# EdwardjkFeng/gradslam

Hardware: AMD Instinct MI355X
Metric: RGB-D frames/sec (640x480, 10 ICP iters) (higher is better)
Workload: dtype f32; 1 GPU; c2: ICP odometry localisation step, 640x480 TUM-shape synthetic RGB-D, batch 1 per GPU, dsratio 4 (~19k x ~19k points), 10 LM iterations, map 288269 points; parallelism=one sequence per GPU, final RCCL all_gather of poses, timing=one timed region of 1356 steps

## Files before the change

gradslam_amd/csrc/gs_icp_assoc.hpp:

```cpp
#pragma once

#include <type_traits>

#include "gs_common.hpp"

namespace gs {

constexpr int KNN_T = 256;
constexpr int KNN_NW = 16;
constexpr int KNN_BT = KNN_NW * 64;
constexpr int KNN_COARSE = 512;
constexpr int CHUNK = 16;
constexpr int WROWS = 3;
constexpr int WBANDS = WROWS + 1;
constexpr int SUPER = 64;
constexpr int KNN_LIST = 4096;
constexpr int NACC = 29;
constexpr int LIN_T = 256;
constexpr int LIN_MAXB = 1024;
constexpr unsigned long long KEY_NONE = ~0ull;

__device__ __forceinline__ unsigned long long pack_key(float d, int j) {
    return ((unsigned long long)fbits(d) << 32) | (unsigned int)j;
}
__device__ __forceinline__ float dist2(f3 s, float tx, float ty, float tz) {
    const float dx = s.x - tx, dy = s.y - ty, dz = s.z - tz;
    return (dx * dx + dy * dy) + dz * dz;
}

struct Row {
    float a[6], b;
    bool valid;
};

__device__ __forceinline__ Row make_row(const float *__restrict__ src, const float *__restrict__ tgt,
                                        const float *__restrict__ nrm, const unsigned long long *__restrict__ best,
                                        int i, int ns, float thresh) {
    Row r;
    r.valid = false;
    if (i >= ns) return r;
    const unsigned long long key = best[i];
    if (key == KEY_NONE) return r;
    const uint32_t j = (uint32_t)(key & 0xffffffffu);
    const float d2 = bitsf((uint32_t)(key >> 32));
    if (thresh >= 0.0f && !(d2 < thresh)) return r;
    const f3 s = ld3(src, i), d = ld3(tgt, j), n = ld3(nrm, j);
    r.a[0] = n.x; r.a[1] = n.y; r.a[2] = n.z;
    r.a[3] = n.z * s.y - n.y * s.z;
    r.a[4] = n.x * s.z - n.z * s.x;
    r.a[5] = n.y * s.x - n.x * s.y;
    r.b = (n.x * (d.x - s.x) + n.y * (d.y - s.y)) + n.z * (d.z - s.z);
    r.valid = true;
    return r;
}

__device__ __forceinline__ void accumulate_row(const Row &r, float *acc) {
    int q = 0;
#pragma unroll
    for (int u = 0; u < 6; ++u)
#pragma unroll
        for (int v = u; v < 6; ++v) { acc[q] = __fmaf_rn(r.a[u], r.a[v], acc[q]); ++q; }
#pragma unroll
    for (int u = 0; u < 6; ++u) acc[21 + u] = __fmaf_rn(r.a[u], r.b, acc[21 + u]);
    acc[27] = __fmaf_rn(r.b, r.b, acc[27]);
    acc[28] += 1.0f;
}

__device__ __forceinline__ Row make_row_from(const f3 s, const bool ok, const unsigned long long key,
                                             const float *__restrict__ tgt, const float *__restrict__ nrm, float thresh) {
    Row r;
    r.valid = false;
    if (!ok || key == KEY_NONE) return r;
    const uint32_t j = (uint32_t)(key & 0xffffffffu);
    const float d2 = bitsf((uint32_t)(key >> 32));
    if (thresh >= 0.0f && !(d2 < thresh)) return r;
    const f3 d = ld3(tgt, j), n = ld3(nrm, j);
    r.a[0] = n.x; r.a[1] = n.y; r.a[2] = n.z;
    r.a[3] = n.z * s.y - n.y * s.z;
    r.a[4] = n.x * s.z - n.z * s.x;
    r.a[5] = n.y * s.x - n.x * s.y;
    r.b = (n.x * (d.x - s.x) + n.y * (d.y - s.y)) + n.z * (d.z - s.z);
    r.valid = true;
    return r;
}

constexpr int POOL = 4096;

struct CamK {
    float R[9], T[3], fx, fy, cx, cy;
    int ds, Wd, Hd;
};
struct KnnShared {
    unsigned long long key[64];
    int cnt;
    float tbox[6];
    int win[WROWS][64];
    int wflag[64];
    int centre[64];
    CamK cam;
    int band[2 * WBANDS + 1];
    int plan[2 * WBANDS];
    unsigned int plan_ready;
    float seed[2][64][4];
    union alignas(16) {
        struct {
            int list[KNN_LIST];
            float rows[NACC][65];
            float part[NACC][16];
        } a;
        float stage[POOL * 4];
    } u;
};

__device__ unsigned int g_loop_counts[4];

#ifdef GS_DIAG_STAMPS
__device__ unsigned long long *g_diag = nullptr;
#define GS_STAMP(slot)                                                                                   \
    do {                                                                                                 \
        if (g_diag && (threadIdx.x & 63) == 0)                                                           \
            g_diag[((size_t)blockIdx.x * KNN_NW + (threadIdx.x >> 6)) * 16 + (slot)] = wall_clock64();   \
    } while (0)
#define GS_COUNT(slot, v)                                                                                \
    do {                                                                                                 \
        if (g_diag && (threadIdx.x & 63) == 0)                                                           \
            g_diag[((size_t)blockIdx.x * KNN_NW + (threadIdx.x >> 6)) * 16 + (slot)] = (v);             \
    } while (0)
#define GS_TICK(var) const unsigned int var = (unsigned int)wall_clock64()
#define GS_ACCUM(acc, t0) acc += (unsigned int)wall_clock64() - (t0)
#else
#define GS_STAMP(slot)
#define GS_COUNT(slot, v)
#define GS_TICK(var)
#define GS_ACCUM(acc, t0)
#endif

__device__ __forceinline__ float rlane(float v, int l) {
    return __int_as_float(__builtin_amdgcn_readlane(__float_as_int(v), l));
}
template <int CTRL>
__device__ __forceinline__ int dpp_i(int v) {
    return __builtin_amdgcn_update_dpp(v, v, CTRL, 0xf, 0xf, false);
}
template <class Op>
__device__ __forceinline__ int wave_reduce_i(int v, Op op) {
    v = op(v, dpp_i<0xB1>(v));
    v = op(v, dpp_i<0x4E>(v));
    v = op(v, dpp_i<0x141>(v));
    v = op(v, dpp_i<0x140>(v));
    return op(op(__builtin_amdgcn_readlane(v, 0), __builtin_amdgcn_readlane(v, 16)),
              op(__builtin_amdgcn_readlane(v, 32), __builtin_amdgcn_readlane(v, 48)));
}
template <class Op>
__device__ __forceinline__ float wave_reduce_f(float v, Op op) {
    auto d = [](float x, auto tag) { return __int_as_float(dpp_i<decltype(tag)::value>(__float_as_int(x))); };
    v = op(v, d(v, std::integral_constant<int, 0xB1>{}));
    v = op(v, d(v, std::integral_constant<int, 0x4E>{}));
    v = op(v, d(v, std::integral_constant<int, 0x141>{}));
    v = op(v, d(v, std::integral_constant<int, 0x140>{}));
    return op(op(rlane(v, 0), rlane(v, 16)), op(rlane(v, 32), rlane(v, 48)));
}
__device__ __forceinline__ float wave_min_f(float v) {
    return wave_reduce_f(v, [](float a, float b) { return fminf(a, b); });
}
__device__ __forceinline__ float wave_max_f(float v) {
    return wave_reduce_f(v, [](float a, float b) { return fmaxf(a, b); });
}

__device__ __forceinline__ void scan_held(const f3 s, const float px, const float py, const float pz, const int pj,
                                          const int n, float &bd, int &bi) {
    for (int k = 0; k < n; ++k) {
        const float d = dist2(s, rlane(px, k), rlane(py, k), rlane(pz, k));
        const int j = __builtin_amdgcn_readlane(pj, k);
        const bool better = (d < bd) | ((d == bd) & (j < bi));
        bd = better ? d : bd;
        bi = better ? j : bi;
    }
}

__device__ __forceinline__ void key_unpack(unsigned long long k, float &bd, int &bi) {
    bd = (k == KEY_NONE) ? INFINITY : bitsf((uint32_t)(k >> 32));
    bi = (k == KEY_NONE) ? 0x7fffffff : (int)(uint32_t)(k & 0xffffffffu);
}

template <int NW>
__device__ __forceinline__ void knn_window_seed(KnnShared &sh, const f3 s, const bool ok, const int i,
                                                const gs_icp_hints &h, const int nt) {
    constexpr int R = 2, WIN = (2 * R + 1) * (2 * R + 1), CAP = 4;
    const int lane = threadIdx.x & 63, wave = threadIdx.x >> 6;
    if (wave == 0) sh.key[lane] = KEY_NONE;
    __syncthreads();
    float bd = INFINITY;
    int bi = 0x7fffffff;
    const int npix = h.grid_w * h.grid_h;
    const int p = ok ? min(max(h.src_pix[i], 0), npix - 1) : 0;
    const int pr = p / h.grid_w, pc = p - pr * h.grid_w;
    for (int wdx = wave; wdx < WIN; wdx += NW) {
        const int rr = pr + wdx / (2 * R + 1) - R, cc = pc + wdx % (2 * R + 1) - R;
        if (!ok || rr < 0 || rr >= h.grid_h || cc < 0 || cc >= h.grid_w) continue;
        const int q0 = rr * h.grid_w + cc;
        const int s0 = h.pix_start[q0], s1 = min(h.pix_start[q0 + 1], s0 + CAP);
        for (int slot = s0; slot < s1; ++slot) {
            const f3 q = ld3(h.scan_points, slot);
            const int oj = h.scan_orig[slot];
            const float d = dist2(s, q.x, q.y, q.z);
            const bool better = (d < bd) | ((d == bd) & (oj < bi));
            bd = better ? d : bd;
            bi = better ? oj : bi;
        }
    }
    if (wave == 0 && ok && bd == INFINITY) {
        const int slot = min(max(h.pix_start[p], 0), nt - 1);
        const f3 q = ld3(h.scan_points, slot);
        bd = dist2(s, q.x, q.y, q.z);
        bi = h.scan_orig[slot];
    }
    if (ok && bd < INFINITY) atomicMin(&sh.key[lane], pack_key(bd, bi));
    __syncthreads();
}

__device__ __forceinline__ void tile_box(KnnShared &sh, const f3 s, const bool act) {
    const int lane = threadIdx.x & 63, wave = threadIdx.x >> 6;
    if (wave >= 1 && wave <= 6) {
        const int a = wave - 1;
        const float v = (a % 3 == 0) ? s.x : ((a % 3 == 1) ? s.y : s.z);
        const float r = (a < 3) ? wave_min_f(act ? v : INFINITY) : wave_max_f(act ? v : -INFINITY);
        if (lane == 0) sh.tbox[a] = r;
    }
}

struct LaneWin {
    __device__ __forceinline__ static int pack(int lo, int n) { return n > 0 ? ((lo / CHUNK) << 9) | ((n + CHUNK - 1) / CHUNK) : 0; }
    __device__ __forceinline__ static int lo(int r) { return (r >> 9) * CHUNK; }
    __device__ __forceinline__ static int len(int r, int nt) { return min((r & 511) * CHUNK, nt - lo(r)); }
    __device__ __forceinline__ static bool covers(const KnnShared &sh, int who, int slot) {
        const int c = slot / CHUNK;
        asm volatile("" : "+v"(who));
        bool in = false;
#pragma unroll
        for (int r = 0; r < WROWS; ++r) {
            const int w = sh.win[r][who];
            in |= (unsigned)(c - (w >> 9)) < (unsigned)(w & 511);
        }
        return in;
    }
};
__device__ __forceinline__ int wave_min_i(int v) {
    return wave_reduce_i(v, [](int a, int b) { return min(a, b); });
}
__device__ __forceinline__ int wave_max_i(int v) {
    return wave_reduce_i(v, [](int a, int b) { return max(a, b); });
}
__device__ __forceinline__ int sel4(int k, int a0, int a1, int a2, int a3) { return k == 0 ? a0 : (k == 1 ? a1 : (k == 2 ? a2 : a3)); }

template <bool GRID, int NW>
__device__ __forceinline__ void knn_prune_search(KnnShared &sh, const f3 s, const bool ok, const bool act,
                                                 const float *__restrict__ scan, const int32_t *__restrict__ scan_orig,
                                                 const float *__restrict__ boxes, const float *__restrict__ sboxes ,
                                                 const int nt) {
    const int lane = threadIdx.x & 63, wave = threadIdx.x >> 6;
    int n_scanned = 0;
    float bd0;
    int bi0;
    key_unpack(sh.key[lane], bd0, bi0);
    const float tlx = sh.tbox[0], tly = sh.tbox[1], tlz = sh.tbox[2];
    const float thx = sh.tbox[3], thy = sh.tbox[4], thz = sh.tbox[5];
    const float bdmax = wave_max_f(act ? bd0 : 0.0f);

    const int nchunks = (nt + CHUNK - 1) / CHUNK;
#ifdef GS_DIAG_STAMPS
    unsigned int t_coarse = 0, t_fine = 0, t_bar = 0, n_tested = 0;
#endif
    for (int r0 = 0; r0 < nchunks; r0 += KNN_LIST) {
        if (threadIdx.x == 0) sh.cnt = 0;
        __syncthreads();
        GS_TICK(tc0);
        const int r1 = min(nchunks, r0 + KNN_LIST);
        for (int c0 = r0 + wave * 64; c0 < r1; c0 += NW * 64) {
            if (sboxes) {
                static_assert(SUPER == 64 && KNN_LIST % SUPER == 0, "one coarse round = one super-box");
                const float *b = sboxes + 6 * (int64_t)__builtin_amdgcn_readfirstlane(c0 / SUPER);
                const float ex = fmaxf(fmaxf(b[0] - thx, tlx - b[3]), 0.0f);
                const float ey = fmaxf(fmaxf(b[1] - thy, tly - b[4]), 0.0f);
                const float ez = fmaxf(fmaxf(b[2] - thz, tlz - b[5]), 0.0f);
                const float lbs = (ex * ex + ey * ey) + ez * ez;
                if (!(lbs <= bdmax)) continue;
            }
            const int c = c0 + lane;
            bool pass = false;
            if (c < r1) {
                const float *b = boxes + 6 * (int64_t)c;
                const float ex = fmaxf(fmaxf(b[0] - thx, tlx - b[3]), 0.0f);
                const float ey = fmaxf(fmaxf(b[1] - thy, tly - b[4]), 0.0f);
                const float ez = fmaxf(fmaxf(b[2] - thz, tlz - b[5]), 0.0f);
                const float lbt = (ex * ex + ey * ey) + ez * ez;
                pass = lbt <= bdmax;
            }
            const unsigned long long m = __ballot(pass);
            if (m) {
                int base = 0;
                if (lane == 0) base = atomicAdd(&sh.cnt, __popcll(m));
                base = __builtin_amdgcn_readfirstlane(base);
                if (pass) sh.u.a.list[base + __popcll(m & ((1ull << lane) - 1ull))] = c;
            }
        }
        GS_ACCUM(t_coarse, tc0);
        GS_TICK(tb0);
        __syncthreads();
        GS_ACCUM(t_bar, tb0);
        GS_TICK(tf0);
        const int nlist = sh.cnt;
        const int ni = (nlist > wave) ? (nlist - wave + NW - 1) / NW : 0;
        constexpr int SEG = 64 / CHUNK;
        for (int g = 0; g < ni; g += SEG) {
            const int seg = lane / CHUNK, idx = g + seg;
            const bool have = idx < ni;
            const int c = have ? sh.u.a.list[wave + NW * idx] : 0;
            const int j = c * CHUNK + (lane % CHUNK);
            const bool pv = have && j < nt;
            const f3 q = pv ? ld3(scan, j) : f3{0.0f, 0.0f, 0.0f};
            const int pj = pv ? (scan_orig ? scan_orig[j] : j) : 0x7fffffff;
            float b0 = 0, b1 = 0, b2 = 0, b3 = 0, b4 = 0, b5 = 0;
            if (have) {
                const float *b = boxes + 6 * (int64_t)c;
                b0 = b[0]; b1 = b[1]; b2 = b[2]; b3 = b[3]; b4 = b[4]; b5 = b[5];
            }
            const int ng = min(SEG, ni - g);
            for (int sg = 0; sg < ng; ++sg) {
                const int l0 = sg * CHUNK;
                float bd;
                int bi;
                key_unpack(sh.key[lane], bd, bi);
                const float ex = fmaxf(fmaxf(rlane(b0, l0) - s.x, s.x - rlane(b3, l0)), 0.0f);
                const float ey = fmaxf(fmaxf(rlane(b1, l0) - s.y, s.y - rlane(b4, l0)), 0.0f);
                const float ez = fmaxf(fmaxf(rlane(b2, l0) - s.z, s.z - rlane(b5, l0)), 0.0f);
                const float lb = (ex * ex + ey * ey) + ez * ez;
                const int cc = __builtin_amdgcn_readlane(c, l0);
                bool hit;
                if (GRID) {
                    const bool live = act & !LaneWin::covers(sh, lane, cc * CHUNK);
                    hit = live & (lb <= bd);
                } else {
                    hit = act & (lb <= bd);
                }
                if (!__any(hit)) continue;
                const int m = min(CHUNK, nt - cc * CHUNK);
                const float bdp = bd;
                const int bip = bi;
                for (int k = 0; k < m; ++k) {
                    const float d = dist2(s, rlane(q.x, l0 + k), rlane(q.y, l0 + k), rlane(q.z, l0 + k));
                    const int jj = __builtin_amdgcn_readlane(pj, l0 + k);
                    const bool better = (d < bd) | ((d == bd) & (jj < bi));
                    bd = better ? d : bd;
                    bi = better ? jj : bi;
                }
                if (ok && (bd < bdp || bi < bip)) atomicMin(&sh.key[lane], pack_key(bd, bi));
                ++n_scanned;
            }
#ifdef GS_DIAG_STAMPS
            n_tested += ng;
#endif
        }
        GS_ACCUM(t_fine, tf0);
        GS_TICK(tb1);
        __syncthreads();
        GS_ACCUM(t_bar, tb1);
    }
    GS_COUNT(8, (unsigned long long)t_coarse);
    GS_COUNT(9, (unsigned long long)t_fine);
    GS_COUNT(10, (unsigned long long)t_bar);
    GS_COUNT(11, (unsigned long long)n_tested);
    GS_COUNT(4, (unsigned long long)n_scanned);
    GS_COUNT(5, (unsigned long long)sh.cnt | ((unsigned long long)__builtin_amdgcn_s_getreg((31 << 11) | 4) << 16) |
                    ((unsigned long long)__builtin_amdgcn_s_getreg((31 << 11) | 20) << 48));
    (void)n_scanned;
}

template <int NW>
__device__ __forceinline__ bool knn_point_search(KnnShared &sh, const f3 s, const unsigned long long need_mask,
                                                 const float *__restrict__ scan, const int32_t *__restrict__ scan_orig,
                                                 const float *__restrict__ boxes, const float *__restrict__ sboxes, const int nt) {
    const int lane = threadIdx.x & 63, wave = threadIdx.x >> 6;
    const int nchunks = (nt + CHUNK - 1) / CHUNK, nsb = (nchunks + SUPER - 1) / SUPER;
    for (unsigned long long rest = need_mask; rest; rest &= rest - 1) {
        const int L = __builtin_ctzll(rest);
        const float px = rlane(s.x, L), py = rlane(s.y, L), pz = rlane(s.z, L);
        float bd;
        int bi;
        key_unpack(sh.key[L], bd, bi);
        for (int b0 = wave * 64; b0 < nsb; b0 += NW * 64) {
            const int sb = b0 + lane;
            bool hit = false;
            if (sb < nsb) {
                const float *b = sboxes + 6 * (int64_t)sb;
                const float ex = fmaxf(fmaxf(b[0] - px, px - b[3]), 0.0f);
                const float ey = fmaxf(fmaxf(b[1] - py, py - b[4]), 0.0f);
                const float ez = fmaxf(fmaxf(b[2] - pz, pz - b[5]), 0.0f);
                const float lb = (ex * ex + ey * ey) + ez * ez;
                hit = lb <= bd;
            }
            const unsigned long long m = __ballot(hit);
            if (m) {
                int base = 0;
                if (lane == 0) base = atomicAdd(&sh.cnt, __popcll(m));
                base = __builtin_amdgcn_readfirstlane(base);
                const int at = base + __popcll(m & ((1ull << lane) - 1ull));
                if (hit && at < KNN_LIST) sh.u.a.list[at] = (L << 24) | sb;
            }
        }
    }
    __syncthreads();
    if (sh.cnt > KNN_LIST) {
        if (threadIdx.x == 0) atomicAdd(&g_loop_counts[3], 1u);
        __syncthreads();
        return false;
    }
    const int npairs = sh.cnt;
    for (int pi = wave; pi < npairs; pi += NW) {
        const int pr = sh.u.a.list[pi];
        const int L = pr >> 24, sb = pr & 0xffffff;
        const f3 p{rlane(s.x, L), rlane(s.y, L), rlane(s.z, L)};
        float bd;
        int bi;
        key_unpack(sh.key[L], bd, bi);
        const int c = sb * SUPER + lane;
        bool hit = false;
        if (c < nchunks && !LaneWin::covers(sh, L, c * CHUNK)) {
            const float *b = boxes + 6 * (int64_t)c;
            const float ex = fmaxf(fmaxf(b[0] - p.x, p.x - b[3]), 0.0f);
            const float ey = fmaxf(fmaxf(b[1] - p.y, p.y - b[4]), 0.0f);
            const float ez = fmaxf(fmaxf(b[2] - p.z, p.z - b[5]), 0.0f);
            const float lb = (ex * ex + ey * ey) + ez * ez;
            hit = lb <= bd;
        }
        unsigned long long hits = __ballot(hit);
        while (hits) {
            constexpr int SEG = 64 / CHUNK;
            int cc = -1;
#pragma unroll
            for (int q = 0; q < SEG; ++q) {
                const int b0 = hits ? __builtin_ctzll(hits) : -1;
                if (hits) hits &= hits - 1;
                if (lane / CHUNK == q) cc = b0;
            }
            unsigned long long k = KEY_NONE;
            if (cc >= 0) {
                const int j = (sb * SUPER + cc) * CHUNK + (lane % CHUNK);
                if (j < nt) {
                    const f3 q = ld3(scan, j);
                    const float d = dist2(p, q.x, q.y, q.z);
                    k = pack_key(d, scan_orig ? scan_orig[j] : j);
                }
            }
#pragma unroll
            for (int off = 32; off > 0; off >>= 1) {
                const unsigned long long o = __shfl_xor(k, off, kWave);
                k = o < k ? o : k;
            }
            if (k < pack_key(bd, bi)) {
                if (lane == 0) atomicMin(&sh.key[L], k);
                key_unpack(k, bd, bi);
            }
        }
    }
    __syncthreads();
    return true;
}

template <int NW>
__device__ __forceinline__ unsigned long long knn_tile(KnnShared &sh, const f3 s, const bool ok, const int seed_j,
                                                       const float *__restrict__ tgt, const float *__restrict__ scan,
                                                       const int32_t *__restrict__ scan_orig,
                                                       const float *__restrict__ boxes, const float *__restrict__ sboxes,
                                                       const int nt) {
    const int lane = threadIdx.x & 63, wave = threadIdx.x >> 6;
    GS_STAMP(0);
    if (wave == 0 && seed_j != -2) {
        unsigned long long k0 = KEY_NONE;
        if (ok && seed_j >= 0) {
            const f3 q = ld3(tgt, seed_j);
            k0 = pack_key(dist2(s, q.x, q.y, q.z), seed_j);
        }
        sh.key[lane] = k0;
    }
    tile_box(sh, s, ok);
    __syncthreads();
    if (seed_j == -1) {
        const int M = min(nt, KNN_COARSE);
        const float stride = (float)nt / (float)M;
        float bd = INFINITY;
        int bi = 0x7fffffff;
        for (int k0 = wave * 16; k0 < M; k0 += NW * 16) {
            const int k = k0 + lane;
            const int n = min(16, M - k0);
            const int j = min((int)((float)k * stride), nt - 1);
            const f3 q = (lane < n) ? ld3(scan, j) : f3{0.0f, 0.0f, 0.0f};
            const int oj = (scan_orig && lane < n) ? scan_orig[j] : j;
            scan_held(s, q.x, q.y, q.z, oj, n, bd, bi);
        }
        if (ok && bd < INFINITY) atomicMin(&sh.key[lane], pack_key(bd, bi));
        __syncthreads();
        if (scan_orig == nullptr) {
        constexpr int R = 64;
        key_unpack(sh.key[lane], bd, bi);
        const int jstar = bi;
        for (int t = 0; t < 2 * R / NW; ++t) {
            const int j = min(max(jstar - R + wave * (2 * R / NW) + t, 0), nt - 1);
            const f3 q = ok ? ld3(tgt, j) : f3{0.0f, 0.0f, 0.0f};
            const float d = dist2(s, q.x, q.y, q.z);
            const bool better = (d < bd) | ((d == bd) & (j < bi));
            bd = better ? d : bd;
            bi = better ? j : bi;
        }
        if (ok && bi != jstar) atomicMin(&sh.key[lane], pack_key(bd, bi));
        __syncthreads();
        }
    }
    GS_STAMP(1);
    knn_prune_search<false, NW>(sh, s, ok, ok, scan, scan_orig, boxes, sboxes, nt);
    GS_STAMP(2);
    GS_STAMP(3);
    return ok ? sh.key[lane] : KEY_NONE;
}

}
```

gradslam_amd/csrc/gs_icp_loop.hpp:

```cpp
#pragma once

#include "gs_icp_step.hpp"
#include "gs_project.hpp"

namespace gs {

struct LoopConst {
    const float *user_src, *tgt, *nrm, *boxes, *sboxes;
    const int32_t *d_ns, *d_nt;
    float *trace, *out_T;
    gs_icp_hints hints;
    GradParams gp;
    float thresh;
    int ns, nt;
    int cert_off;
    int tile_points;
    int grid_variant;
    CamK cam;
    int cam_ok;
    int32_t *cells;
    int cells_stride;
};

__device__ __forceinline__ f3 cam_point(const CamK &k, const f3 p) {
    return f3{dot3_fma(p.x, p.y, p.z, k.R[0], k.R[3], k.R[6]) + k.T[0],
              dot3_fma(p.x, p.y, p.z, k.R[1], k.R[4], k.R[7]) + k.T[1],
              dot3_fma(p.x, p.y, p.z, k.R[2], k.R[5], k.R[8]) + k.T[2]};
}
__device__ __forceinline__ int cam_cell(const CamK &k, const f3 p) {
    const f3 q = cam_point(k, p);
    const float zs = (q.z != 0.0f) ? q.z : 1.0f;
    const float ds = (float)k.ds;
    const float u = ((k.fx * q.x + k.cx * q.z) / zs) / ds, v = ((k.fy * q.y + k.cy * q.z) / zs) / ds;
    const int cc = (int)fminf(fmaxf(rintf(u), 0.0f), (float)(k.Wd - 1));
    const int cr = (int)fminf(fmaxf(rintf(v), 0.0f), (float)(k.Hd - 1));
    return cr * k.Wd + cc;
}
__device__ __forceinline__ float cam_bound2(const CamK &k, const f3 s, const int centre, const int R) {
    const f3 q = cam_point(k, s);
    const int cr = centre / k.Wd, cc = centre - cr * k.Wd;
    const float ds = (float)k.ds;
    const float hw = (float)(R + 1) * ds - 0.52f;
    const float uc = (float)cc * ds, vc = (float)cr * ds;
    float L = INFINITY;
    if (cc + R + 1 < k.Wd) { const float a = k.cx - (uc + hw); L = fminf(L, -(k.fx * q.x + a * q.z) * __builtin_amdgcn_rsqf(k.fx * k.fx + a * a)); }
    if (cc - R - 1 >= 0) { const float a = k.cx - (uc - hw); L = fminf(L, (k.fx * q.x + a * q.z) * __builtin_amdgcn_rsqf(k.fx * k.fx + a * a)); }
    if (cr + R + 1 < k.Hd) { const float a = k.cy - (vc + hw); L = fminf(L, -(k.fy * q.y + a * q.z) * __builtin_amdgcn_rsqf(k.fy * k.fy + a * a)); }
    if (cr - R - 1 >= 0) { const float a = k.cy - (vc - hw); L = fminf(L, (k.fy * q.y + a * q.z) * __builtin_amdgcn_rsqf(k.fy * k.fy + a * a)); }
    L = L * 0.998f - 1e-5f;
    return L > 0.0f ? L * L : 0.0f;
}

template <bool GRID, int NL, int NW>
__global__ __launch_bounds__(NW * 64, 2 * NW / 4) void knn1_loop_k(const LoopConst *__restrict__ C, const IcpState *__restrict__ S_in,
                                                         const float *__restrict__ partials_in, const int32_t *__restrict__ pix_ws,
                                                         const int32_t *__restrict__ cells_in, int cap, int tile_points,
                                                         int phase , int step_mode, int look_slot,
                                                         int nblocks_in, IcpState *__restrict__ S_out, float *__restrict__ rec, int out_slot,
                                                         LoopBufs B, float *__restrict__ partials ,
                                                         const float *__restrict__ user_src) {
    static_assert(NW == 16 || NW == 8, "row groups, tile_box and the J epilogue are laid out for sixteen or eight waves");
    const int first = phase & 1, par = phase >> 1;
    __shared__ KnnShared sh;
    __shared__ IcpState st_sm;
    __shared__ float acc_sm[NACC];
    __shared__ double lu_sm[42];
    constexpr int kWords = sizeof(IcpState) / 4;
    GS_STAMP(6);
    const int lane = threadIdx.x & 63, wave = threadIdx.x >> 6;
    const int tile0 = blockIdx.x * tile_points;
    const int i = tile0 + lane;
    constexpr bool grid = GRID;
    __shared__ unsigned int rp_cnt;
    if constexpr (GRID) {
        if (threadIdx.x == 0) { rp_cnt = 0; sh.plan_ready = 0; }
        if (wave == 0) __builtin_amdgcn_s_waitcnt(0xc07f);
        __builtin_amdgcn_s_barrier();
    }
    const int ic = min(i, cap - 1);
    const int st_w = reinterpret_cast<const int *>(S_in)[min((int)threadIdx.x, kWords - 1)];
    float rp_a[RP_LOADS];
    int rp_g, rp_g2, rp_g3 = -1;
    if constexpr (NW == 16) {
        rp_g = (GRID && (wave == 1 || wave == 2)) ? -1 : (int)(threadIdx.x >> 5);
        rp_g2 = (GRID && wave >= 14) ? (int)(threadIdx.x >> 5) - 26 : -1;
    } else if constexpr (GRID) {
        const int tg = threadIdx.x >> 5, w = tg < 2 ? tg : tg - 4;
        const bool sums = wave != 1 && wave != 2;
        rp_g = sums ? w : -1;
        rp_g2 = sums ? w + 12 : -1;
        rp_g3 = (sums && w < 8) ? w + 24 : -1;
    } else {
        rp_g = threadIdx.x >> 5;
        rp_g2 = rp_g + 16;
    }
    float rp_b[RP_LOADS], rp_c[RP_LOADS];
#pragma unroll
    for (int u = 0; u < RP_LOADS; ++u) { rp_a[u] = 0.0f; rp_b[u] = 0.0f; rp_c[u] = 0.0f; }
    if (rp_g >= 0) rp_issue_padded<NL>(partials_in, rp_g, rp_a);
    if (rp_g2 >= 0) rp_issue_padded<NL>(partials_in, rp_g2, rp_b);
    if constexpr (NW != 16 && GRID) {
        if (rp_g3 >= 0) rp_issue_padded<NL>(partials_in, rp_g3, rp_c);
    }
    static_assert(offsetof(LoopConst, nt) == offsetof(LoopConst, ns) + 4, "ns | nt are read as a pair");
    const int nn = reinterpret_cast<const int *>(&C->ns)[lane & 1];
    int e_h = 0, e_c = -1, e_cam = 0;
    unsigned long long e_k0 = 0, e_k1 = 0;
    if constexpr (GRID) {
        e_h = pix_ws[ic];
        e_c = cells_in[ic];
        const int ik = wave == 2 ? ic : 0;
        e_k0 = B.N(0)[ik]; e_k1 = B.N(1)[ik];
        e_cam = reinterpret_cast<const int *>(&C->cam)[min(lane, (int)(sizeof(CamK) / 4) - 1)];
        asm volatile("" ::"v"(e_h), "v"(e_c), "v"(e_cam), "v"((unsigned)e_k0), "v"((unsigned)(e_k0 >> 32)),
                     "v"((unsigned)e_k1), "v"((unsigned)(e_k1 >> 32)));
    }
    if constexpr (NW != 16 && GRID)
        asm volatile("" ::"v"(rp_c[0]), "v"(rp_c[1]), "v"(rp_c[2]), "v"(rp_c[3]), "v"(rp_c[4]), "v"(rp_c[5]), "v"(rp_c[6]), "v"(rp_c[7]), "v"(rp_c[8]),
                     "v"(rp_c[9]), "v"(rp_c[10]), "v"(rp_c[11]), "v"(rp_c[12]), "v"(rp_c[13]), "v"(rp_c[14]), "v"(rp_c[15]));
    if constexpr (GRID || NW != 16)
        asm volatile("" ::"v"(rp_b[0]), "v"(rp_b[1]), "v"(rp_b[2]), "v"(rp_b[3]), "v"(rp_b[4]), "v"(rp_b[5]), "v"(rp_b[6]), "v"(rp_b[7]), "v"(rp_b[8]),
                     "v"(rp_b[9]), "v"(rp_b[10]), "v"(rp_b[11]), "v"(rp_b[12]), "v"(rp_b[13]), "v"(rp_b[14]), "v"(rp_b[15]));
    asm volatile("" ::"v"(st_w), "v"(nn), "v"(rp_a[0]), "v"(rp_a[1]), "v"(rp_a[2]), "v"(rp_a[3]), "v"(rp_a[4]), "v"(rp_a[5]), "v"(rp_a[6]),
                 "v"(rp_a[7]), "v"(rp_a[8]), "v"(rp_a[9]), "v"(rp_a[10]), "v"(rp_a[11]), "v"(rp_a[12]), "v"(rp_a[13]), "v"(rp_a[14]),
                 "v"(rp_a[15]));
    GS_STAMP(8);
    const int ns = __builtin_amdgcn_readlane(nn, 0), nt = __builtin_amdgcn_readlane(nn, 1);
    const bool ok = lane < tile_points && i < ns;
    const bool tile_live = tile0 < ns && nt > 0;
    if (tile0 >= ns && blockIdx.x != 0) {
        if (threadIdx.x < NACC) partials[blockIdx.x * NACC + threadIdx.x] = 0.0f;
        return;
    }
    f3 e_pp{0.0f, 0.0f, 0.0f};
    unsigned long long e_ka = 0, e_kb = 0;
    if (GRID && grid && tile_live && wave != 0 && ok) {
        if (first && C->cam_ok) e_pp = ld3(user_src, i);
        if (wave == 2 && !first) {
            const int ba = S_in->b_cur;
            if (look_slot < 0) { e_ka = ba == 0 ? e_k0 : e_k1; e_kb = ba == 0 ? e_k1 : e_k0; }
            else { e_ka = B.N(ba)[i]; e_kb = B.N(look_slot)[i]; }
        }
    }

    if (threadIdx.x < kWords) reinterpret_cast<int *>(&st_sm)[threadIdx.x] = st_w;
    if (step_mode >= 0) {
        if constexpr (GRID) {
            float v = 0.0f, v2 = 0.0f, v3 = 0.0f;
            if (rp_g >= 0) v = rp_sum_padded<NL>(rp_a);
            if (rp_g2 >= 0) v2 = rp_sum_padded<NL>(rp_b);
            if constexpr (NW != 16) {
                if (rp_g3 >= 0) v3 = rp_sum_padded<NL>(rp_c);
            }
            rp_finish_wave0<NW>(v, rp_g, v2, rp_g2, v3, rp_g3, acc_sm, &rp_cnt);
        } else if constexpr (NW == 16) {
            rp_finish(rp_sum_padded<NL>(rp_a), acc_sm);
        } else {
            rp_finish2(rp_sum_padded<NL>(rp_a), rp_sum_padded<NL>(rp_b), acc_sm);
        }
        GS_STAMP(9);
        if (blockIdx.x == 0 && rec && threadIdx.x < kWords) reinterpret_cast<int *>(rec)[REC_STATE + threadIdx.x] = st_w;
    }
    if (wave == 0) {
        const bool pub = blockIdx.x == 0;
        if (step_mode >= 0)
            step_wave0(&st_sm, acc_sm, step_mode, C->gp, pub ? C->trace : nullptr, pub ? C->out_T : nullptr, look_slot, pub ? rec : nullptr, lu_sm, true);
        GS_STAMP(10);
    } else if (!grid && tile_live && !first && wave == 1) {
        if (ok) {
            const int ba = S_in->b_cur, bb = look_slot >= 0 ? look_slot : 1 - ba;
            const unsigned long long ka = B.N(ba)[i], kb = B.N(bb)[i];
            const int sa = (int)min((uint32_t)(ka & 0xffffffffu), (uint32_t)(nt - 1)), sb = (int)min((uint32_t)(kb & 0xffffffffu), (uint32_t)(nt - 1));
            const f3 qa = ld3(C->tgt, sa), qb = ld3(C->tgt, sb);
            *reinterpret_cast<float4 *>(sh.seed[0][lane]) = make_float4(qa.x, qa.y, qa.z, __int_as_float(sa));
            *reinterpret_cast<float4 *>(sh.seed[1][lane]) = make_float4(qb.x, qb.y, qb.z, __int_as_float(sb));
        }
    } else if (grid && tile_live) {
        const int Wd = C->hints.grid_w, nc = C->hints.grid_w * C->hints.grid_h;
        constexpr int R = 1;
        int bbase[WBANDS], pstart[WBANDS], bcnt[WBANDS], used = 0;
#pragma unroll
        for (int q = 0; q < WBANDS; ++q) { bbase[q] = 0; pstart[q] = 0x7fffffff; bcnt[q] = 0; }
        const int h = ok ? min(max(e_h, 0), nc - 1) : 0;
        int c = h;
        if (wave <= 2 && ok && C->cam_ok) c = first ? cam_cell(C->cam, xform(S_in->dT, e_pp)) : min(max(e_c, 0), nc - 1);
        int row_lo[WROWS], row_hi[WROWS];
        float4 sd[2] = {make_float4(0.0f, 0.0f, 0.0f, 0.0f), make_float4(0.0f, 0.0f, 0.0f, 0.0f)};
#pragma unroll
        for (int r = 0; r < WROWS; ++r) { row_lo[r] = 0; row_hi[r] = 0; }
        if (wave == 2) {
#pragma unroll
            for (int r = 0; r < WROWS; ++r) {
                const int g = c + (r - 1) * Wd;
                row_lo[r] = C->hints.pix_start[min(max(g - 1, 0), nc - 1)];
                row_hi[r] = C->hints.pix_start[min(max(g + 1, 0), nc - 1) + 1];
            }
            if (ok) {
                int sj[2];
                if (first) {
                    const int slot = min(max(C->hints.pix_start[h], 0), nt - 1);
                    sj[0] = sj[1] = min(max(C->hints.scan_orig[slot], 0), nt - 1);
                } else {
                    sj[0] = (int)min((uint32_t)(e_ka & 0xffffffffu), (uint32_t)(nt - 1));
                    sj[1] = (int)min((uint32_t)(e_kb & 0xffffffffu), (uint32_t)(nt - 1));
                }
#pragma unroll
                for (int u = 0; u < 2; ++u) {
                    const f3 q = ld3(C->tgt, sj[u]);
                    sd[u] = make_float4(q.x, q.y, q.z, __int_as_float(sj[u]));
                }
            }
        }
        if (wave == 1) {
            const int dsp = c - h;
            auto near = [&](int r) { return abs(r) <= 3 || abs(r - Wd) <= 3 || abs(r + Wd) <= 3; };
            const unsigned long long okm = __ballot(ok);
            unsigned long long pool = okm, sup = 0;
            for (int tries = 0; tries < 3 && pool; ++tries) {
                const int cand = __builtin_amdgcn_readlane(dsp, __builtin_ctzll(pool));
                const unsigned long long m = __ballot(ok && near(dsp - cand));
                if (__popcll(m) > __popcll(sup)) sup = m;
                if (2 * __popcll(m) >= __popcll(okm)) break;
                pool &= ~m;
            }
            GS_STAMP(13);
            const bool mine = ok && ((sup >> lane) & 1);
            const int dmin = __builtin_amdgcn_readfirstlane(wave_min_i(mine ? dsp : 0x7fffffff));
            const int e = mine ? dsp - dmin : 0;
            int rel = mine ? (e >= Wd / 2) + (e >= Wd + Wd / 2) : 2;
            const bool in = mine && rel <= 1 && abs(e - rel * Wd) <= 6;
            if (!in) rel = 2;
            const int beta = c - rel * Wd;
            const int bmin = __builtin_amdgcn_readfirstlane(wave_min_i(in ? beta : 0x7fffffff));
            const int bmax = __builtin_amdgcn_readfirstlane(wave_max_i(in ? beta : (int)0x80000000));
            const bool two_rows = __any(in && rel == 1);
            int boff[WBANDS];
            {
                int lo_raw[WBANDS], hi_raw[WBANDS];
                bool want[WBANDS];
#pragma unroll
                for (int kk = 0; kk < WBANDS; ++kk) {
                    const int a = bmin + (kk - R) * Wd - R, b = bmax + (kk - R) * Wd + R;
                    want[kk] = kk <= 2 * R + (two_rows ? 1 : 0) && bmax >= bmin && b >= 0 && a <= nc - 1;
                    lo_raw[kk] = C->hints.pix_start[min(max(a, 0), nc - 1)];
                    hi_raw[kk] = C->hints.pix_start[min(max(b, 0), nc - 1) + 1];
                }
                sh.centre[lane] = c;
                sh.wflag[lane] = rel;
#pragma unroll
                for (int kk = 0; kk < WBANDS; ++kk) {
                    bbase[kk] = 0; bcnt[kk] = 0; boff[kk] = used;
                    const int lo = min(max(lo_raw[kk], 0), nt) & ~(CHUNK - 1);
                    const int hi = min((min(max(hi_raw[kk], 0), nt) + CHUNK - 1) & ~(CHUNK - 1), nt);
                    if (want[kk] && hi > lo) {
                        bbase[kk] = lo; bcnt[kk] = hi - lo;
                        if (used + (hi - lo) <= POOL) used += hi - lo; else boff[kk] = -1;
                    }
                }
            }
            if (lane < WBANDS) {
                int bb = bbase[0], bo = boff[0], bn = bcnt[0];
#pragma unroll
                for (int q = 1; q < WBANDS; ++q) { bb = lane == q ? bbase[q] : bb; bo = lane == q ? boff[q] : bo; bn = lane == q ? bcnt[q] : bn; }
                sh.band[lane] = bb; sh.band[WBANDS + lane] = bo;
                sh.plan[lane] = (bo >= 0 && bn > 0) ? bo : 0x7fffffff;
                sh.plan[WBANDS + lane] = bn;
            }
            if (lane == 0) { sh.band[2 * WBANDS] = used; sh.cnt = 0; }
            sh.key[lane] = KEY_NONE;
            if (lane == 0) __hip_atomic_store(&sh.plan_ready, 1u, __ATOMIC_RELEASE, __HIP_MEMORY_SCOPE_WORKGROUP);
#pragma unroll
            for (int q = 0; q < WBANDS; ++q) pstart[q] = (boff[q] >= 0 && bcnt[q] > 0) ? boff[q] : 0x7fffffff;
        } else {
            while (__hip_atomic_load(&sh.plan_ready, __ATOMIC_ACQUIRE, __HIP_MEMORY_SCOPE_WORKGROUP) == 0u) __builtin_amdgcn_s_sleep(2);
            const int pl = sh.band[min(lane, 2 * WBANDS)], ps = sh.plan[min(lane, 2 * WBANDS - 1)];
#pragma unroll
            for (int q = 0; q < WBANDS; ++q) {
                bbase[q] = __builtin_amdgcn_readlane(pl, q);
                pstart[q] = __builtin_amdgcn_readlane(ps, q);
                bcnt[q] = __builtin_amdgcn_readlane(ps, WBANDS + q);
            }
            used = __builtin_amdgcn_readlane(pl, 2 * WBANDS);
        }
        GS_STAMP(14);
        constexpr int ST = NW * 64 - 64, NR = (POOL + ST - 1) / ST;
        float4 sreg[NR];
#pragma unroll
        for (int r = 0; r < NR; ++r) {
            const int e = (int)threadIdx.x - 64 + ST * r;
            if (e < used) {
                int bb = 0, bo = 0;
#pragma unroll
                for (int q = 0; q < WBANDS; ++q) {
                    const bool here = e >= pstart[q];
                    bb = here ? bbase[q] : bb; bo = here ? pstart[q] : bo;
                }
                const int slot = bb + e - bo;
                const f3 q3 = ld3(C->hints.scan_points, slot);
                sreg[r] = make_float4(q3.x, q3.y, q3.z, __int_as_float(C->hints.scan_orig[slot]));
            }
        }
        if (wave == 2) {
            const int rel = sh.wflag[lane];
            const bool in = rel <= 1;
            bool full = in;
#pragma unroll
            for (int r = 0; r < WROWS; ++r) {
                int packed = 0;
                const int g = c + (r - R) * Wd;
                if (in && r <= 2 * R && g + R >= 0 && g - R <= nc - 1) {
                    const int lo = min(max(row_lo[r], 0), nt) & ~(CHUNK - 1);
                    const int hi = min((min(max(row_hi[r], 0), nt) + CHUNK - 1) & ~(CHUNK - 1), nt);
                    if (hi > lo) {
                        int bb = bbase[0], bn = bcnt[0];
#pragma unroll
                        for (int q = 1; q < WBANDS; ++q) { bb = (rel + r) == q ? bbase[q] : bb; bn = (rel + r) == q ? bcnt[q] : bn; }
                        if (lo >= bb && hi <= bb + bn && (hi - lo + CHUNK - 1) / CHUNK <= 511) packed = LaneWin::pack(lo, hi - lo); else full = false;
                    }
                }
                sh.win[r][lane] = packed;
            }
            sh.wflag[lane] = min(rel, 2) | (full ? 4 : 0) | (R << 3);
            if (lane < (int)(sizeof(CamK) / 4)) reinterpret_cast<int *>(&sh.cam)[lane] = e_cam;
            *reinterpret_cast<float4 *>(sh.seed[0][lane]) = sd[0];
            *reinterpret_cast<float4 *>(sh.seed[1][lane]) = sd[1];
        }
#pragma unroll
        for (int r = 0; r < NR; ++r) {
            const int e = (int)threadIdx.x - 64 + ST * r;
            if (e < used) *reinterpret_cast<float4 *>(&sh.u.stage[4 * e]) = sreg[r];
        }
        GS_STAMP(15);
    }
    __syncthreads();
    if (step_mode >= 0 && blockIdx.x == 0 && threadIdx.x < kWords) {
        const int v = reinterpret_cast<const int *>(&st_sm)[threadIdx.x];
        reinterpret_cast<int *>(S_out)[threadIdx.x] = v;
        if (rec) reinterpret_cast<int *>(rec)[REC_WORDS + REC_STATE + threadIdx.x] = v;
    }
    GS_STAMP(7);
    const IcpState *S = &st_sm;
    if (tile0 >= ns) {
        if (threadIdx.x < NACC) partials[blockIdx.x * NACC + threadIdx.x] = 0.0f;
        return;
    }
    const int p_cur = S->p_cur, b_cur = S->b_cur;
    const float *in = first ? user_src : B.P(p_cur);
    float *out = B.P(out_slot >= 0 ? out_slot : 1 - p_cur);
    unsigned long long *best = B.N(out_slot >= 0 ? out_slot : 1 - b_cur);
    f3 s{0.0f, 0.0f, 0.0f};
    if (ok) {
        s = xform(S->dT, ld3(in, i));
        if (wave == 0) st3(out, i, s);
    }
    if (nt <= 0) {
        if (ok && wave == 0) best[i] = KEY_NONE;
        if (threadIdx.x < NACC) partials[blockIdx.x * NACC + threadIdx.x] = 0.0f;
        return;
    }
    unsigned long long key;
    bool need = false;
    int rel = 2;
    if (grid) {
        GS_STAMP(0);
        rel = sh.wflag[lane];
        if (wave == 0) {
            unsigned long long k0 = KEY_NONE;
            if (ok) {
                const int u = (first || b_cur == S_in->b_cur) ? 0 : 1;
                const float4 q = *reinterpret_cast<const float4 *>(sh.seed[u][lane]);
                k0 = pack_key(dist2(s, q.x, q.y, q.z), __float_as_int(q.w));
            }
            atomicMin(&sh.key[lane], k0);
        }
        {
            float bd = INFINITY;
            int bi = 0x7fffffff;
#pragma unroll
            for (int r = 0; r < WROWS; ++r) {
                const int wr = sh.win[r][lane];
                const int kk = (rel & 3) + r, wn = LaneWin::len(wr, nt);
                const int po = sh.band[WBANDS + min(kk, WBANDS - 1)];
                const float *row = sh.u.stage + 4 * (max(po, 0) + LaneWin::lo(wr) - sh.band[min(kk, WBANDS - 1)]);
                for (int p = wave; p < wn; p += NW) {
                    float4 q;
                    if (po >= 0) {
                        q = *reinterpret_cast<const float4 *>(row + 4 * p);
                    } else {
                        const int slot = LaneWin::lo(wr) + p;
                        const f3 g3 = ld3(C->hints.scan_points, slot);
                        q = make_float4(g3.x, g3.y, g3.z, __int_as_float(C->hints.scan_orig[slot]));
                    }
                    const float d = dist2(s, q.x, q.y, q.z);
                    const int jj = __float_as_int(q.w);
                    const bool better = (d < bd) | ((d == bd) & (jj < bi));
                    bd = better ? d : bd;
                    bi = better ? jj : bi;
                }
            }
            if (ok && bd < INFINITY) atomicMin(&sh.key[lane], pack_key(bd, bi));
        }
        __syncthreads();
        GS_STAMP(1);
        float bd;
        int bi;
        key_unpack(sh.key[lane], bd, bi);
        const float bound2 = (ok && C->cam_ok) ? cam_bound2(sh.cam, s, sh.centre[lane], rel >> 3) : 0.0f;
        const bool proven = !C->cert_off & ((rel & 4) != 0) & (bd * 1.0001f < bound2);
        need = ok & !proven;
        const unsigned long long need_mask = __ballot(need);
        GS_COUNT(12, (unsigned long long)__popcll(need_mask));
        bool tile_search = __popcll(need_mask) > 6;
        if (!tile_search && need_mask) {
            tile_search = !knn_point_search<NW>(sh, s, need_mask, C->hints.scan_points, C->hints.scan_orig, C->boxes, C->sboxes, nt);
        }
        if (tile_search) {
            tile_box(sh, s, need);
            __syncthreads();
            knn_prune_search<true, NW>(sh, s, ok, need, C->hints.scan_points, C->hints.scan_orig, C->boxes, C->sboxes, nt);
        }
        GS_STAMP(2);
        key = ok ? sh.key[lane] : KEY_NONE;
        GS_STAMP(3);
        GS_COUNT(5, ((unsigned long long)__builtin_amdgcn_s_getreg((31 << 11) | 4) << 16) |
                        ((unsigned long long)__builtin_amdgcn_s_getreg((31 << 11) | 20) << 48));
    } else {
        int sj = -1;
        if (!first) {
            sj = -2;
            if (wave == 0) {
                unsigned long long k0 = KEY_NONE;
                if (ok) {
                    const float4 q = *reinterpret_cast<const float4 *>(sh.seed[b_cur == S_in->b_cur ? 0 : 1][lane]);
                    k0 = pack_key(dist2(s, q.x, q.y, q.z), __float_as_int(q.w));
                }
                sh.key[lane] = k0;
            }
        }
        const bool window_seed = first && C->hints.scan_points && C->hints.src_pix && C->hints.pix_start && C->hints.grid_w > 0;
        if (window_seed) sj = -2;
        const float *scan = C->hints.scan_points ? C->hints.scan_points : C->tgt;
        const int32_t *scan_orig = C->hints.scan_points ? C->hints.scan_orig : nullptr;
        if (window_seed) knn_window_seed<NW>(sh, s, ok, i, C->hints, nt);
        key = knn_tile<NW>(sh, s, ok, sj, C->tgt, scan, scan_orig, C->boxes, C->sboxes, nt);
    }
    if (wave == 0) {
        if (ok) best[i] = key;
        if (grid && ok && C->cam_ok) C->cells[par * C->cells_stride + i] = cam_cell(sh.cam, s);
        float acc[NACC];
#pragma unroll
        for (int k = 0; k < NACC; ++k) acc[k] = 0.0f;
        const Row r = make_row_from(s, ok, key, C->tgt, C->nrm, C->thresh);
        if (r.valid) accumulate_row(r, acc);
#pragma unroll
        for (int k = 0; k < NACC; ++k) sh.u.a.rows[k][lane] = acc[k];
    }
    __syncthreads();
    static_assert(NACC * 16 <= NW * 64, "the J epilogue's first stage is one pass");
    if (threadIdx.x < NACC * 16) {
        const int k = threadIdx.x >> 4, p4 = (threadIdx.x & 15) * 4;
        sh.u.a.part[k][threadIdx.x & 15] = ((sh.u.a.rows[k][p4] + sh.u.a.rows[k][p4 + 1]) + sh.u.a.rows[k][p4 + 2]) + sh.u.a.rows[k][p4 + 3];
    }
    __syncthreads();
    if (threadIdx.x < NACC) {
        float v = 0.0f;
#pragma unroll
        for (int q = 0; q < 16; ++q) v += sh.u.a.part[threadIdx.x][q];
        partials[blockIdx.x * NACC + threadIdx.x] = v;
    }
}

__global__ void icp_init_state_k(IcpState *S, const float *__restrict__ init_T , float damp) {
    if (threadIdx.x == 0 && blockIdx.x == 0) {
        for (int i = 0; i < 16; ++i) {
            const float v = init_T ? init_T[i] : ((i % 5 == 0) ? 1.0f : 0.0f);
            S->T[i] = v; S->dT[i] = v;
        }
        for (int i = 0; i < 44; ++i) S->cur[i] = 0.0f;
        S->damp = damp;
        S->p_cur = 1;
        S->b_cur = 1; S->b_first = 0;
        S->it = 0;
    }
}

__global__ __launch_bounds__(SUPER * CHUNK) void icp_prepare_k(IcpState *S, const float *__restrict__ init_T, float damp,
                                                              const float *__restrict__ tgt, const int32_t *__restrict__ d_nt,
                                                              float *__restrict__ boxes, float *__restrict__ sboxes,
                                                              LoopConst lc, LoopConst *__restrict__ lc_out, float *__restrict__ part0,
                                                              float *__restrict__ part1, int rows_written, int rows_read) {
    static_assert(SUPER * CHUNK == 1024, "one block per super-box");
    for (int q = rows_written * NACC + blockIdx.x * blockDim.x + threadIdx.x; q < rows_read * NACC; q += gridDim.x * blockDim.x) {
        part0[q] = 0.0f; part1[q] = 0.0f;
    }
    __shared__ float wb[16][6];
    if (blockIdx.x == 0 && threadIdx.x < sizeof(LoopConst) / 4) {
        int v = reinterpret_cast<const int *>(&lc)[threadIdx.x];
        if (threadIdx.x == offsetof(LoopConst, ns) / 4) v = *lc.d_ns;
        if (threadIdx.x == offsetof(LoopConst, nt) / 4) v = *lc.d_nt;
        if (threadIdx.x == offsetof(LoopConst, tile_points) / 4) {
            atomicAdd(&g_loop_counts[0], 1u);
            if (lc.grid_variant) atomicAdd(&g_loop_counts[1], 1u);
            if (lc.tile_points != 64) atomicAdd(&g_loop_counts[2], 1u);
        }
        reinterpret_cast<int *>(lc_out)[threadIdx.x] = v;
    }
    if (lc.cells) {
        const int n = *lc.d_ns;
        int32_t *pix = lc.cells + 2 * (size_t)lc.cells_stride;
        for (int i = blockIdx.x * blockDim.x + threadIdx.x; i < lc.cells_stride; i += gridDim.x * blockDim.x)
            pix[i] = (i < n && lc.hints.src_pix) ? lc.hints.src_pix[i] : 0;
    }
    if (blockIdx.x == 0) {
        __syncthreads();
        if (threadIdx.x == 0 && lc.hints.cam_pose && lc.hints.cam_K && lc.hints.ds > 0) {
            const float *T = lc.hints.cam_pose, *K = lc.hints.cam_K;
            const Cam c = make_cam(T, K);
            for (int q = 0; q < 9; ++q) lc_out->cam.R[q] = c.R[q];
            for (int q = 0; q < 3; ++q) lc_out->cam.T[q] = c.tinv[q];
            lc_out->cam.fx = K[0]; lc_out->cam.fy = K[5]; lc_out->cam.cx = K[2]; lc_out->cam.cy = K[6];
            lc_out->cam.ds = lc.hints.ds; lc_out->cam.Wd = lc.hints.grid_w; lc_out->cam.Hd = lc.hints.grid_h;
            const bool pinhole = K[1] == 0.0f && K[3] == 0.0f && K[4] == 0.0f && K[7] == 0.0f && K[8] == 0.0f && K[9] == 0.0f &&
                                 K[10] == 1.0f && K[11] == 0.0f && K[0] != 0.0f && K[5] != 0.0f;
            lc_out->cam_ok = pinhole ? 1 : 0;
        }
    }
    if (threadIdx.x == 0 && blockIdx.x == 0) {
        for (int i = 0; i < 16; ++i) {
            const float v = init_T ? init_T[i] : ((i % 5 == 0) ? 1.0f : 0.0f);
            S->T[i] = v; S->dT[i] = v;
        }
        for (int i = 0; i < 44; ++i) S->cur[i] = 0.0f;
        for (int i = 0; i < 6; ++i) S->xi[i] = 0.0f;
        S->damp = damp;
        S->p_cur = 1;
        S->b_cur = 1; S->b_first = 0;
        S->it = 0;
    }
    const int nt = *d_nt;
    const int j = blockIdx.x * (SUPER * CHUNK) + threadIdx.x;
    if (blockIdx.x * (SUPER * CHUNK) >= nt) return;
    float lo[3] = {INFINITY, INFINITY, INFINITY}, hi[3] = {-INFINITY, -INFINITY, -INFINITY};
    if (j < nt) {
        const f3 p = ld3(tgt, j);
        lo[0] = hi[0] = p.x; lo[1] = hi[1] = p.y; lo[2] = hi[2] = p.z;
    }
#pragma unroll
    for (int a = 0; a < 3; ++a) {
#pragma unroll
        for (int off = CHUNK / 2; off > 0; off >>= 1) {
            lo[a] = fminf(lo[a], __shfl_xor(lo[a], off, kWave));
            hi[a] = fmaxf(hi[a], __shfl_xor(hi[a], off, kWave));
        }
    }
    if ((threadIdx.x % CHUNK) == 0 && j < nt) {
        float *b = boxes + 6 * (int64_t)(j / CHUNK);
        b[0] = lo[0]; b[1] = lo[1]; b[2] = lo[2]; b[3] = hi[0]; b[4] = hi[1]; b[5] = hi[2];
    }
#pragma unroll
    for (int a = 0; a < 3; ++a) {
#pragma unroll
        for (int off = 32; off >= CHUNK; off >>= 1) {
            lo[a] = fminf(lo[a], __shfl_xor(lo[a], off, kWave));
            hi[a] = fmaxf(hi[a], __shfl_xor(hi[a], off, kWave));
        }
    }
    const int lane = threadIdx.x & 63, wave = threadIdx.x >> 6;
    if (lane == 0) { wb[wave][0] = lo[0]; wb[wave][1] = lo[1]; wb[wave][2] = lo[2]; wb[wave][3] = hi[0]; wb[wave][4] = hi[1]; wb[wave][5] = hi[2]; }
    __syncthreads();
    if (threadIdx.x < 6) {
        float v = wb[0][threadIdx.x];
        for (int w = 1; w < 16; ++w) v = threadIdx.x < 3 ? fminf(v, wb[w][threadIdx.x]) : fmaxf(v, wb[w][threadIdx.x]);
        sboxes[6 * (int64_t)blockIdx.x + threadIdx.x] = v;
    }
}

__global__ void copy_best_last_k(const IcpState *__restrict__ S, LoopBufs B, const int32_t *__restrict__ d_ns,
                                 unsigned long long *__restrict__ out) {
    const unsigned long long *src = B.N(S->b_first);
    const int ns = *d_ns;
    for (int i = blockIdx.x * blockDim.x + threadIdx.x; i < ns; i += gridDim.x * blockDim.x) out[i] = src[i];
}

}
```

Before: 5563 frames/s.

## Prefetch source points and target/normal rows early in eight-wave grid ICP kernel

```diff
diff --git a/gradslam_amd/csrc/gs_icp_assoc.hpp b/gradslam_amd/csrc/gs_icp_assoc.hpp
--- a/gradslam_amd/csrc/gs_icp_assoc.hpp
+++ b/gradslam_amd/csrc/gs_icp_assoc.hpp
@@ -75,6 +75,28 @@
     const float d2 = bitsf((uint32_t)(key >> 32));
     if (thresh >= 0.0f && !(d2 < thresh)) return r;
     const f3 d = ld3(tgt, j), n = ld3(nrm, j);
+    r.a[0] = n.x; r.a[1] = n.y; r.a[2] = n.z;
+    r.a[3] = n.z * s.y - n.y * s.z;
+    r.a[4] = n.x * s.z - n.z * s.x;
+    r.a[5] = n.y * s.x - n.x * s.y;
+    r.b = (n.x * (d.x - s.x) + n.y * (d.y - s.y)) + n.z * (d.z - s.z);
+    r.valid = true;
+    return r;
+}
+
+__device__ __forceinline__ f3 ld3_global(const float *p, int64_t i) {
+    const __attribute__((address_space(1))) float *q = (const __attribute__((address_space(1))) float *)(p + 3 * i);
+    return f3{q[0], q[1], q[2]};
+}
+__device__ __forceinline__ Row make_row_with(const f3 s, const bool ok, const unsigned long long key, const bool have, const f3 d0,
+                                             const f3 n0, const float *__restrict__ tgt, const float *__restrict__ nrm, float thresh) {
+    Row r;
+    r.valid = false;
+    if (!ok || key == KEY_NONE) return r;
+    const uint32_t j = (uint32_t)(key & 0xffffffffu);
+    const float d2 = bitsf((uint32_t)(key >> 32));
+    if (thresh >= 0.0f && !(d2 < thresh)) return r;
+    const f3 d = have ? d0 : ld3(tgt, j), n = have ? n0 : ld3(nrm, j);
     r.a[0] = n.x; r.a[1] = n.y; r.a[2] = n.z;
     r.a[3] = n.z * s.y - n.y * s.z;
     r.a[4] = n.x * s.z - n.z * s.x;
diff --git a/gradslam_amd/csrc/gs_icp_loop.hpp b/gradslam_amd/csrc/gs_icp_loop.hpp
--- a/gradslam_amd/csrc/gs_icp_loop.hpp
+++ b/gradslam_amd/csrc/gs_icp_loop.hpp
@@ -71,6 +71,7 @@
     const int tile0 = blockIdx.x * tile_points;
     const int i = tile0 + lane;
     constexpr bool grid = GRID;
+    constexpr bool behind = GRID && NW == 8;
     __shared__ unsigned int rp_cnt;
     if constexpr (GRID) {
         if (threadIdx.x == 0) { rp_cnt = 0; sh.plan_ready = 0; }
@@ -106,12 +107,17 @@
     const int nn = reinterpret_cast<const int *>(&C->ns)[lane & 1];
     int e_h = 0, e_c = -1, e_cam = 0;
     unsigned long long e_k0 = 0, e_k1 = 0;
+    f3 e_p0{0.0f, 0.0f, 0.0f}, e_p1{0.0f, 0.0f, 0.0f};
     if constexpr (GRID) {
         e_h = pix_ws[ic];
         e_c = cells_in[ic];
         const int ik = wave == 2 ? ic : 0;
         e_k0 = B.N(0)[ik]; e_k1 = B.N(1)[ik];
         e_cam = reinterpret_cast<const int *>(&C->cam)[min(lane, (int)(sizeof(CamK) / 4) - 1)];
+        if constexpr (behind) {
+            e_p0 = ld3(B.P(0), ic); e_p1 = ld3(B.P(1), ic);
+            asm volatile("" ::"v"(e_p0.x), "v"(e_p0.y), "v"(e_p0.z), "v"(e_p1.x), "v"(e_p1.y), "v"(e_p1.z));
+        }
         asm volatile("" ::"v"(e_h), "v"(e_c), "v"(e_cam), "v"((unsigned)e_k0), "v"((unsigned)(e_k0 >> 32)),
                      "v"((unsigned)e_k1), "v"((unsigned)(e_k1 >> 32)));
     }
@@ -134,8 +140,8 @@
     }
     f3 e_pp{0.0f, 0.0f, 0.0f};
     unsigned long long e_ka = 0, e_kb = 0;
-    if (GRID && grid && tile_live && wave != 0 && ok) {
-        if (first && C->cam_ok) e_pp = ld3(user_src, i);
+    if (GRID && grid && tile_live && (behind || wave != 0) && ok) {
+        if (first && (behind || C->cam_ok)) e_pp = ld3(user_src, i);
         if (wave == 2 && !first) {
             const int ba = S_in->b_cur;
             if (look_slot < 0) { e_ka = ba == 0 ? e_k0 : e_k1; e_kb = ba == 0 ? e_k1 : e_k0; }
@@ -161,8 +167,12 @@
         GS_STAMP(9);
         if (blockIdx.x == 0 && rec && threadIdx.x < kWords) reinterpret_cast<int *>(rec)[REC_STATE + threadIdx.x] = st_w;
     }
+    int b_old = -1;
     if (wave == 0) {
         const bool pub = blockIdx.x == 0;
+        if constexpr (behind) {
+            if (step_mode >= 0) b_old = st_sm.b_cur;
+        }
         if (step_mode >= 0)
             step_wave0(&st_sm, acc_sm, step_mode, C->gp, pub ? C->trace : nullptr, pub ? C->out_T : nullptr, look_slot, pub ? rec : nullptr, lu_sm, true);
         GS_STAMP(10);
@@ -350,7 +360,14 @@
     unsigned long long *best = B.N(out_slot >= 0 ? out_slot : 1 - b_cur);
     f3 s{0.0f, 0.0f, 0.0f};
     if (ok) {
-        s = xform(S->dT, ld3(in, i));
+        f3 p;
+        if constexpr (behind) {
+            if (first ? tile_live : (p_cur == 0 || p_cur == 1)) p = first ? e_pp : (p_cur == 0 ? e_p0 : e_p1);
+            else p = ld3(in, i);
+        } else {
+            p = ld3(in, i);
+        }
+        s = xform(S->dT, p);
         if (wave == 0) st3(out, i, s);
     }
     if (nt <= 0) {
@@ -358,7 +375,7 @@
         if (threadIdx.x < NACC) partials[blockIdx.x * NACC + threadIdx.x] = 0.0f;
         return;
     }
-    unsigned long long key;
+    unsigned long long key, wkey = KEY_NONE;
     bool need = false;
     int rel = 2;
     if (grid) {
@@ -367,13 +384,62 @@
         if (wave == 0) {
             unsigned long long k0 = KEY_NONE;
             if (ok) {
-                const int u = (first || b_cur == S_in->b_cur) ? 0 : 1;
+                int u;
+                if constexpr (behind) u = (first || step_mode < 0 || b_cur == b_old) ? 0 : 1;
+                else u = (first || b_cur == S_in->b_cur) ? 0 : 1;
                 const float4 q = *reinterpret_cast<const float4 *>(sh.seed[u][lane]);
                 k0 = pack_key(dist2(s, q.x, q.y, q.z), __float_as_int(q.w));
             }
             atomicMin(&sh.key[lane], k0);
         }
-        {
+        bool scanned = false;
+        if constexpr (behind) {
+            const int w3[WROWS] = {sh.win[0][lane], sh.win[1][lane], sh.win[2][lane]};
+            int bw[2 * WBANDS];
+#pragma unroll
+            for (int q = 0; q < 2 * WBANDS; ++q) bw[q] = sh.band[q];
+            if (__builtin_amdgcn_readfirstlane(bw[WBANDS] | bw[WBANDS + 1] | bw[WBANDS + 2] | bw[WBANDS + 3]) >= 0) {
+                scanned = true;
+                static_assert(WROWS == 3 && WBANDS == 4, "the batched scan is written out for three rows in four bands");
+                int rb[WROWS], wn[WROWS];
+#pragma unroll
+                for (int r = 0; r < WROWS; ++r) {
+                    const int kk = min((rel & 3) + r, WBANDS - 1);
+                    rb[r] = sel4(kk, bw[4], bw[5], bw[6], bw[7]) + LaneWin::lo(w3[r]) - sel4(kk, bw[0], bw[1], bw[2], bw[3]);
+                    wn[r] = LaneWin::len(w3[r], nt);
+                }
+                constexpr int RB = 2;
+                const float4 *pool = reinterpret_cast<const float4 *>(sh.u.stage);
+                const int wmax = max(wn[0], max(wn[1], wn[2]));
+                float bd = INFINITY;
+                int bi = 0x7fffffff;
+                for (int p0 = wave; __any(p0 < wmax); p0 += RB * NW) {
+                    float4 q[WROWS][RB];
+#pragma unroll
+                    for (int r = 0; r < WROWS; ++r)
+#pragma unroll
+                        for (int t = 0; t < RB; ++t) {
+                            const int p = p0 + t * NW;
+                            q[r][t] = pool[p < wn[r] ? rb[r] + p : 0];
+                        }
+#pragma unroll
+                    for (int r = 0; r < WROWS; ++r)
+#pragma unroll
+                        for (int t = 0; t < RB; ++t) {
+                            const bool have = p0 + t * NW < wn[r];
+                            float d = dist2(s, q[r][t].x, q[r][t].y, q[r][t].z);
+                            asm volatile("" : "+v"(d));
+                            d = have ? d : INFINITY;
+                            const int jj = have ? __float_as_int(q[r][t].w) : 0x7fffffff;
+                            const bool better = (d < bd) | ((d == bd) & (jj < bi));
+                            bd = better ? d : bd;
+                            bi = better ? jj : bi;
+                        }
+                }
+                if (ok && bd < INFINITY) atomicMin(&sh.key[lane], pack_key(bd, bi));
+            }
+        }
+        if (!scanned) {
             float bd = INFINITY;
             int bi = 0x7fffffff;
 #pragma unroll
@@ -404,7 +470,12 @@
         GS_STAMP(1);
         float bd;
         int bi;
-        key_unpack(sh.key[lane], bd, bi);
+        wkey = sh.key[lane];
+        key_unpack(wkey, bd, bi);
+        if constexpr (behind) {
+            const uint32_t jg = wave == 0 ? min((uint32_t)bi, (uint32_t)(nt - 1)) : 0u;
+            e_p0 = ld3_global(C->tgt, jg); e_p1 = ld3_global(C->nrm, jg);
+        }
         const float bound2 = (ok && C->cam_ok) ? cam_bound2(sh.cam, s, sh.centre[lane], rel >> 3) : 0.0f;
         const bool proven = !C->cert_off & ((rel & 4) != 0) & (bd * 1.0001f < bound2);
         need = ok & !proven;
@@ -450,7 +521,8 @@
         float acc[NACC];
 #pragma unroll
         for (int k = 0; k < NACC; ++k) acc[k] = 0.0f;
-        const Row r = make_row_from(s, ok, key, C->tgt, C->nrm, C->thresh);
+        const Row r = behind ? make_row_with(s, ok, key, key == wkey, e_p0, e_p1, C->tgt, C->nrm, C->thresh)
+                             : make_row_from(s, ok, key, C->tgt, C->nrm, C->thresh);
         if (r.valid) accumulate_row(r, acc);
 #pragma unroll
         for (int k = 0; k < NACC; ++k) sh.u.a.rows[k][lane] = acc[k];
```

Measured after the change: 5646 frames/s, median of 6. +1.5%, better.
